# YyzHarry/imbalanced-regression

Measured on NVIDIA H100. Metric: images/sec, higher is better.
Workload: dtype bf16

## Files before the change

imbalanced-regression_b200/csrc/common.cuh:

```cuda
#pragma once
#include <cuda_runtime.h>
#include <cuda_bf16.h>
#include <stdint.h>
#include <stdio.h>
#include <stdlib.h>
#include <atomic>
#include <vector>
#include "../../include/dirb200.h"

namespace dirb200 {

void set_error(const char* fmt, ...);
extern std::atomic<int64_t> g_launches;

inline cudaStream_t as_stream(void* s) { return reinterpret_cast<cudaStream_t>(s); }

#define DIRB_CHECK_ARG(cond, ...)                \
  do {                                           \
    if (!(cond)) {                               \
      ::dirb200::set_error(__VA_ARGS__);         \
      return DIRB200_ERR_ARG;                    \
    }                                            \
  } while (0)

// ... 12 lines not shown
    DIRB_CUDA(cudaGetLastError());                \
  } while (0)

inline int num_sms() {
  static int n = 0;
  if (n == 0) {
    int dev = 0;
    if (cudaGetDevice(&dev) != cudaSuccess) return 132;
    if (cudaDeviceGetAttribute(&n, cudaDevAttrMultiProcessorCount, dev) != cudaSuccess || n <= 0) n = 132;
    if (const char* e = getenv("DIRB200_SMS")) {
      const int cap = atoi(e);
      if (cap > 0 && cap < n) n = cap;
    }
  }
  return n;
}

__device__ __forceinline__ float warp_sum(float v) {
#pragma unroll
  for (int o = 16; o > 0; o >>= 1) v += __shfl_xor_sync(0xffffffffu, v, o);
  return v;
}
__device__ __forceinline__ double warp_sum(double v) {
#pragma unroll
  for (int o = 16; o > 0; o >>= 1) v += __shfl_xor_sync(0xffffffffu, v, o);
  return v;
}

struct FastDiv {
  uint32_t mul, shr, d;
// ... 44 lines not shown
```

imbalanced-regression_b200/csrc/conv.cuh:

```cuda
#pragma once
#include "common.cuh"

namespace dirb200 {

struct ConvShape {
  int n, h, w, cin, cout, kh, kw, stride, pad, ho, wo;
};

struct StatLayout {
  int rows, n_tiles, bn, group;
};

int conv_fprop(const __nv_bfloat16* x, const __nv_bfloat16* w, __nv_bfloat16* y, const ConvShape& s, bool stem,
               cudaStream_t st, float* stat_partial = nullptr, StatLayout* layout = nullptr);
struct ConvEpilogue {
  const float* scale;
  const float* shift;
  const __nv_bfloat16* residual;
  bool relu;
};
int conv_fprop_affine(const __nv_bfloat16* x, const __nv_bfloat16* w, __nv_bfloat16* out, const ConvShape& s,
                      const ConvEpilogue& epi, cudaStream_t st);
struct DgradBnMoments {
  const __nv_bfloat16* y;
// ... 10 lines not shown
                        int* splits_out, cudaStream_t st);
int wgrad_reduce(const float* workspace, int splits, float* dw, const ConvShape& s, bool stem, bool accumulate,
                 cudaStream_t st);
int conv_wgrad(const __nv_bfloat16* x, const __nv_bfloat16* dy, float* dw, float* workspace, const ConvShape& s,
               bool stem, bool accumulate, cudaStream_t st);
struct WgradReduceDesc {
  const float* partial;
  size_t w_off;
  int splits, cout, cin, kh, kw, stem;
};
int wgrad_reduce_all(const WgradReduceDesc* descs_dev, int nlayers, float* grads, cudaStream_t st);
struct PrepDesc {
  size_t w_off;
  int cout, cin, kh, kw, stem;
  __nv_bfloat16 *wf, *wd;
  FastDiv fd_cin, fd_cout, fd_taps;
};
inline PrepDesc make_prep_desc(size_t w_off, int cout, int cin, int kh, int kw, int stem, __nv_bfloat16* wf,
                               __nv_bfloat16* wd) {
  PrepDesc d{w_off, cout, cin, kh, kw, stem, wf, wd, {}, {}, {}};
  d.fd_cin = make_fastdiv((uint32_t)cin);
  d.fd_cout = make_fastdiv((uint32_t)cout);
  d.fd_taps = make_fastdiv((uint32_t)(kh * kw));
  return d;
}
int conv_plan(const ConvShape& s, bool stem, int op, int* plan);
int prep_weights_all(const float* params, const PrepDesc* descs_dev, int nlayers, cudaStream_t st);
int prep_weights(const float* w, int cout, int cin, int kh, int kw, bool stem, __nv_bfloat16* wf, __nv_bfloat16* wd,
                 cudaStream_t st);
int input_to_s2d(const float* x, int n, int h, int w, __nv_bfloat16* out, cudaStream_t st);

}
```

imbalanced-regression_b200/csrc/conv_api.cu:

```cuda
#include "common.cuh"
#include "conv.cuh"

namespace dirb200 {

__global__ void prep_weights_kernel(const float* __restrict__ w, int cout, int cin, int kh, int kw,
                                    __nv_bfloat16* __restrict__ wf, __nv_bfloat16* __restrict__ wd) {
  const int64_t total = (int64_t)cout * cin * kh * kw;
  for (int64_t i = blockIdx.x * (int64_t)blockDim.x + threadIdx.x; i < total; i += (int64_t)gridDim.x * blockDim.x) {
    int c = (int)(i % cin);
    int64_t t = i / cin;
    int s = (int)(t % kw); t /= kw;
    int r = (int)(t % kh);
    int co = (int)(t / kh);
    const float v = w[(((int64_t)co * cin + c) * kh + r) * kw + s];
    const __nv_bfloat16 b = __float2bfloat16_rn(v);
    wf[i] = b;
    if (wd) wd[(((int64_t)c * kh + r) * kw + s) * cout + co] = b;
  }
}

__global__ void prep_stem_weights_kernel(const float* __restrict__ w, int cout, __nv_bfloat16* __restrict__ wf) {
  const int total = cout * 256;
  for (int i = blockIdx.x * blockDim.x + threadIdx.x; i < total; i += gridDim.x * blockDim.x) {
    const int co = i >> 8, k = i & 255;
    const int rp = k >> 6, sp = (k >> 4) & 3, ph = (k >> 3) & 1, pw = (k >> 2) & 1, c = k & 3;
    const int r = 2 * rp + ph - 1, s = 2 * sp + pw - 1;
    float v = 0.f;
    if (c < 3 && r >= 0 && s >= 0 && r < 7 && s < 7) v = w[((co * 3 + c) * 7 + r) * 7 + s];
    wf[i] = __float2bfloat16_rn(v);
  }
}

__global__ void input_to_s2d_kernel(const float* __restrict__ x, int n, int h, int w, __nv_bfloat16* __restrict__ out) {
  const int h2 = h / 2, w2 = w / 2;
  const int64_t total = (int64_t)n * h2 * w2;
  for (int64_t i = blockIdx.x * (int64_t)blockDim.x + threadIdx.x; i < total; i += (int64_t)gridDim.x * blockDim.x) {
    const int xw = (int)(i % w2);
    const int yh = (int)((i / w2) % h2);
    const int b = (int)(i / ((int64_t)w2 * h2));
    __align__(16) __nv_bfloat16 v[16];
#pragma unroll
    for (int ph = 0; ph < 2; ++ph)
#pragma unroll
      for (int pw = 0; pw < 2; ++pw) {
#pragma unroll
        for (int c = 0; c < 3; ++c)
          v[(ph * 2 + pw) * 4 + c] =
              __float2bfloat16_rn(x[(((int64_t)b * 3 + c) * h + (2 * yh + ph)) * w + (2 * xw + pw)]);
// ... 26 lines not shown
  const int total = 256 * cout;
  for (int i = blockIdx.x * blockDim.x + threadIdx.x; i < total; i += gridDim.x * blockDim.x) {
    const int co = i >> 8, k = i & 255;
    const int rp = k >> 6, sp_ = (k >> 4) & 3, ph = (k >> 3) & 1, pw = (k >> 2) & 1, c = k & 3;
    const int r = 2 * rp + ph - 1, s = 2 * sp_ + pw - 1;
    if (c >= 3 || r < 0 || s < 0) continue;
    float acc = 0.f;
    for (int sp = 0; sp < splits; ++sp) acc += partial[(int64_t)sp * total + i];
    float* o = dw + ((co * 3 + c) * 7 + r) * 7 + s;
    *o = accumulate ? *o + acc : acc;
  }
}

__global__ void __launch_bounds__(256)
wgrad_reduce_all_kernel(const WgradReduceDesc* __restrict__ descs, float* __restrict__ grads) {
  const WgradReduceDesc d = descs[blockIdx.y];
  float* dw = grads + d.w_off;
  if (d.stem) {
    const int total = 256 * d.cout;
    for (int i = blockIdx.x * blockDim.x + threadIdx.x; i < total; i += gridDim.x * blockDim.x) {
      const int co = i >> 8, k = i & 255;
      const int rp = k >> 6, sp_ = (k >> 4) & 3, ph = (k >> 3) & 1, pw = (k >> 2) & 1, c = k & 3;
      const int r = 2 * rp + ph - 1, s = 2 * sp_ + pw - 1;
      if (c >= 3 || r < 0 || s < 0) continue;
      float acc = 0.f;
      for (int sp = 0; sp < d.splits; ++sp) acc += d.partial[(int64_t)sp * total + i];
      dw[((co * 3 + c) * 7 + r) * 7 + s] += acc;
    }
    return;
  }
// ... 7 lines not shown
    for (; sp + 4 <= d.splits; sp += 4) {
      a0 += p[(int64_t)sp * total];
      a1 += p[(int64_t)(sp + 1) * total];
      a2 += p[(int64_t)(sp + 2) * total];
      a3 += p[(int64_t)(sp + 3) * total];
    }
    for (; sp < d.splits; ++sp) a0 += p[(int64_t)sp * total];
    const int64_t co = i / ktot, k = i - co * ktot;
    const int c = (int)(k % d.cin), t = (int)(k / d.cin);
    dw[(co * d.cin + c) * taps + t] += (a0 + a1) + (a2 + a3);
  }
}

int wgrad_reduce_all(const WgradReduceDesc* descs_dev, int nlayers, float* grads, cudaStream_t st) {
  if (nlayers <= 0) return DIRB200_OK;
  wgrad_reduce_all_kernel<<<dim3(2 * num_sms(), nlayers), 256, 0, st>>>(descs_dev, grads);
  DIRB_LAUNCHED();
  return DIRB200_OK;
}

__global__ void prep_weights_all_kernel(const float* __restrict__ params, const PrepDesc* __restrict__ descs) {
  const PrepDesc d = descs[blockIdx.y];
  const float* w = params + d.w_off;
  if (d.stem) {
    const int total = d.cout * 256;
    for (int i = blockIdx.x * blockDim.x + threadIdx.x; i < total; i += gridDim.x * blockDim.x) {
      const int co = i >> 8, k = i & 255;
      const int rp = k >> 6, sp = (k >> 4) & 3, ph = (k >> 3) & 1, pw = (k >> 2) & 1, c = k & 3;
      const int r = 2 * rp + ph - 1, s = 2 * sp + pw - 1;
      float v = 0.f;
      if (c < 3 && r >= 0 && s >= 0 && r < 7 && s < 7) v = w[((co * 3 + c) * 7 + r) * 7 + s];
      d.wf[i] = __float2bfloat16_rn(v);
    }
    return;
  }
  const uint32_t taps = (uint32_t)(d.kh * d.kw);
  const uint32_t total = (uint32_t)d.cout * (uint32_t)d.cin * taps;
  const uint32_t stride = gridDim.x * blockDim.x;
  for (uint32_t i = blockIdx.x * blockDim.x + threadIdx.x; i < total; i += stride) {
    uint32_t t, c, co, tap;
    d.fd_cin.divmod(i, t, c);
    d.fd_taps.divmod(t, co, tap);
    d.wf[i] = __float2bfloat16_rn(w[((size_t)co * d.cin + c) * taps + tap]);
  }
  if (!d.wd) return;
  for (uint32_t i = blockIdx.x * blockDim.x + threadIdx.x; i < total; i += stride) {
    uint32_t t, c, co, tap;
    d.fd_cout.divmod(i, t, co);
    d.fd_taps.divmod(t, c, tap);
    d.wd[i] = __float2bfloat16_rn(w[((size_t)co * d.cin + c) * taps + tap]);
  }
}

int prep_weights_all(const float* params, const PrepDesc* descs_dev, int nlayers, cudaStream_t st) {
  prep_weights_all_kernel<<<dim3(96, nlayers), 256, 0, st>>>(params, descs_dev);
  DIRB_LAUNCHED();
  return DIRB200_OK;
}

static inline int grid1d(int64_t n, int block = 256) {
  int64_t g = (n + block - 1) / block;
  const int64_t cap = 8 * (int64_t)num_sms();
  return (int)(g < 1 ? 1 : (g > cap ? cap : g));
}

int prep_weights(const float* w, int cout, int cin, int kh, int kw, bool stem, __nv_bfloat16* wf, __nv_bfloat16* wd,
                 cudaStream_t st) {
  if (stem) {
    prep_stem_weights_kernel<<<grid1d((int64_t)cout * 256), 256, 0, st>>>(w, cout, wf);
  } else {
    prep_weights_kernel<<<grid1d((int64_t)cout * cin * kh * kw), 256, 0, st>>>(w, cout, cin, kh, kw, wf, wd);
  }
  DIRB_LAUNCHED();
  return DIRB200_OK;
}

int input_to_s2d(const float* x, int n, int h, int w, __nv_bfloat16* out, cudaStream_t st) {
  input_to_s2d_kernel<<<grid1d((int64_t)n * (h / 2) * (w / 2)), 256, 0, st>>>(x, n, h, w, out);
  DIRB_LAUNCHED();
  return DIRB200_OK;
}

int wgrad_reduce(const float* workspace, int splits, float* dw, const ConvShape& s, bool stem, bool accumulate,
                 cudaStream_t st) {
  if (stem)
    wgrad_reduce_stem_kernel<<<grid1d(256 * (int64_t)s.cout), 256, 0, st>>>(workspace, splits, s.cout, accumulate, dw);
  else
  {
    const int64_t total = (int64_t)s.kh * s.kw * s.cin * s.cout;
    wgrad_reduce_kernel<<<(unsigned)((total + 255) / 256), 256, 0, st>>>(workspace, splits, s.cout, s.cin, s.kh, s.kw,
                                                                         accumulate, dw);
  }
  DIRB_LAUNCHED();
// ... 181 lines not shown
```

imbalanced-regression_b200/csrc/conv_igemm.cu:

```cuda
#include <stdlib.h>
#include "common.cuh"
#include "tc.cuh"
#include "conv.cuh"

namespace dirb200 {
using namespace tc;

constexpr int BM = 128;
constexpr int BK = 64;
constexpr int kProducerThreads = 128;
constexpr int kThreads = 384;
constexpr int kMaxTaps = 25;
constexpr int kMaxSmemBytes = 232448;

struct IgemmParams {
  const __nv_bfloat16* src;
  int n, hs, ws, cs;
  int hm, wm;
  int kh, kw, stride, pad;
  int transposed;
  int cls_on, cls_py, cls_px, full_h, full_w;
  int ntaps_c;
  int tap_list[kMaxTaps];
  long long tap_eoff[kMaxTaps];
// ... 133 lines not shown
    } else {
      split = 0;
      m_tile = t;
      n_tile = fixed_n;
      kb_begin = 0;
      nk = P.num_kblocks;
    }
  };

  if (threadIdx.x == 0) {
    for (int s = 0; s < C::kStages; ++s) {
      mbar_init(full_bar(s), ATMA ? 1 : kProducerThreads + 1);
      mbar_init(empty_bar(s), 8);
    }
    fence_barrier_init();
  }
  __syncthreads();

  if (warp < 4) {
    if constexpr (!ATMA) {
      const int j = lane & 7;
      const int q = lane >> 3;
      uint32_t rs = 0, rph = 0;
      for (int t = tile_first; t < tile_end; t += tile_step) {
        int split, m_tile, n_tile, kb_begin, nk;
        decode_tile(t, split, m_tile, n_tile, kb_begin, nk);
        const int n0 = n_tile * BN;
        long long off8[8];
        uint32_t mask8[8];
        int chunk_r = 0, chunk_s = 0, chunk_c0 = 0;
        bool chunk_ok = true;
        uint32_t tile_off = 0;
// ... 478 lines not shown
}

template <int BN, bool WGRAD, bool STEM, bool ATMA = false, bool AFFINE = false, bool BSTAT = false>
static int launch_igemm_impl(const CUtensorMap& tm, const CUtensorMap& tma, const IgemmParams& Qin, cudaStream_t st) {
  using C = Cfg<BN, !WGRAD>;
  const IgemmParams Q = finish_params(Qin);
  static bool configured = false;
  if (!configured) {
    DIRB_CUDA(cudaFuncSetAttribute(igemm_kernel<BN, WGRAD, STEM, ATMA, AFFINE, BSTAT>,
                                   cudaFuncAttributeMaxDynamicSharedMemorySize, C::kSmemBytes));
    configured = true;
  }
  int grid = Q.num_tiles < num_sms() ? Q.num_tiles : num_sms();
  if (!WGRAD && grid < Q.n_tiles) grid = Q.n_tiles;
  t_last_layout = StatLayout{grid, Q.n_tiles, BN, 1};
  igemm_kernel<BN, WGRAD, STEM, ATMA, AFFINE, BSTAT><<<grid, kThreads, C::kSmemBytes, st>>>(tm, tma, Q);
  DIRB_LAUNCHED();
  return DIRB200_OK;
}

template <int BN, bool WGRAD, bool STEM>
static int launch_igemm(const CUtensorMap& tm, const IgemmParams& P, int m_tiles, int splits, cudaStream_t st,
                        const CUtensorMap* tma = nullptr) {
  IgemmParams Q = P;
  Q.m_tiles = m_tiles;
  Q.num_tiles = m_tiles * P.n_tiles * splits;
  if constexpr (!STEM) {
    if (tma) {
      if constexpr (!WGRAD) {
        if (Q.epi_scale != nullptr) return launch_igemm_impl<BN, false, false, true, true>(tm, *tma, Q, st);
        if (Q.bst_y != nullptr) return launch_igemm_impl<BN, false, false, true, false, true>(tm, *tma, Q, st);
// ... 313 lines not shown
```

imbalanced-regression_b200/csrc/nn_kernels.cu:

```cuda
#include "common.cuh"
#include "conv.cuh"
#include "nn.cuh"

namespace dirb200 {

constexpr int kReduceCtasPerSm = 4;

struct V8 {
  float v[8];
};
__device__ __forceinline__ V8 load8(const __nv_bfloat16* p) {
  const uint4 u = *reinterpret_cast<const uint4*>(p);
  const __nv_bfloat162* h = reinterpret_cast<const __nv_bfloat162*>(&u);
  V8 r;
#pragma unroll
  for (int i = 0; i < 4; ++i) {
    const float2 f = __bfloat1622float2(h[i]);
    r.v[2 * i] = f.x;
    r.v[2 * i + 1] = f.y;
  }
  return r;
}
__device__ __forceinline__ void store8(__nv_bfloat16* p, const V8& a) {
  uint4 u;
// ... 122 lines not shown
  sh[1][threadIdx.y][threadIdx.x] = b0 + b1;
  __syncthreads();
  r0 = r1 = 0.0;
  if (threadIdx.y == 0)
    for (int w = 0; w < 32; ++w) {
      r0 += sh[0][w][threadIdx.x];
      r1 += sh[1][w][threadIdx.x];
    }
}

__global__ void bn_finalize_kernel(const float* __restrict__ partial, StatLayout L, int64_t rows, int c,
                                   const float* __restrict__ gamma, const float* __restrict__ beta, float eps,
                                   float momentum, float* __restrict__ running_mean, float* __restrict__ running_var,
                                   float* __restrict__ mean_out, float* __restrict__ invstd_out,
                                   float* __restrict__ scale, float* __restrict__ shift) {
  __shared__ double sh[2][32][32];
  const int i = blockIdx.x * 32 + threadIdx.x;
  double sx, sq;
  sum_layout2(partial, L, c, i, sh, sx, sq);
  if (threadIdx.y != 0 || i >= c) return;
  const double n = (double)rows;
  const double m = sx / n;
  double var = sq / n - m * m;
  if (var < 0.0) var = 0.0;
  const float invstd = (float)(1.0 / sqrt(var + (double)eps));
  mean_out[i] = (float)m;
  invstd_out[i] = invstd;
  const float sc = gamma[i] * invstd;
  scale[i] = sc;
  shift[i] = beta[i] - (float)m * sc;
// ... 23 lines not shown
  d.scale[i] = sc;
  d.shift[i] = params[d.beta_off + i] - running[d.rm_off + i] * sc;
}

__device__ __forceinline__ uint32_t f2_to_bf2(float a, float b) {
  __nv_bfloat162 h = __floats2bfloat162_rn(a, b);
  return *reinterpret_cast<uint32_t*>(&h);
}

template <bool HAS_RES, bool HAS_RESY, bool MASK>
__global__ void __launch_bounds__(256)
bn_apply_kernel(const __nv_bfloat16* __restrict__ y, const float* __restrict__ scale, const float* __restrict__ shift,
                const __nv_bfloat16* __restrict__ res, const __nv_bfloat16* __restrict__ res_y,
                const float* __restrict__ res_scale, const float* __restrict__ res_shift, int relu, int64_t rows,
                int c, __nv_bfloat16* __restrict__ out, uint8_t* __restrict__ mask_out) {
  constexpr int R = (HAS_RES || HAS_RESY) ? 2 : 4;
  const int cgroups = c / 8;
  const int cg = threadIdx.x % cgroups, lane = threadIdx.x / cgroups, lanes = blockDim.x / cgroups;
  const V8 sc = loadf8(scale + cg * 8), sh = loadf8(shift + cg * 8);
  V8 rs{}, rh{};
  if (HAS_RESY) {
    rs = loadf8(res_scale + cg * 8);
    rh = loadf8(res_shift + cg * 8);
  }
  const int64_t stride = (int64_t)gridDim.x * lanes;
  for (int64_t r0 = blockIdx.x * (int64_t)lanes + lane; r0 < rows; r0 += R * stride) {
    int64_t offs[R], rr[R];
    bool live[R];
    uint4 Y[R], RV[R];
#pragma unroll
// ... 80 lines not shown
    hw.divmod(static_cast<uint32_t>(r), n, rem);
    w.divmod(rem, yy, xx);
    r2 = (static_cast<int64_t>(n) * h2 + (yy >> 1)) * w2 + (xx >> 1);
    return ((yy | xx) & 1u) == 0u;
  }
};

template <int MODE, int G2M, bool HAS_Y2, bool WRITE_DZ, bool HAS_G3 = false>
__global__ void __launch_bounds__(256, 3)
bn_bwd_reduce_kernel(const __nv_bfloat16* __restrict__ g1, const __nv_bfloat16* __restrict__ g2, CompactG2 cg2,
                     const __nv_bfloat16* __restrict__ g3, const __nv_bfloat16* __restrict__ y,
                     const __nv_bfloat16* __restrict__ y2,
                     const float* __restrict__ scale, const float* __restrict__ shift,
                     const uint8_t* __restrict__ mask, int64_t rows, int c, float* __restrict__ partial,
                     __nv_bfloat16* __restrict__ dz_out) {
  constexpr bool HAS_G2 = G2M != G2_NONE;
  const int cgroups = c / 8;
  const int cg = threadIdx.x % cgroups, lane = threadIdx.x / cgroups, lanes = blockDim.x / cgroups;
  constexpr int K = HAS_Y2 ? 3 : 2;
  float acc[K][8] = {};
  MaskSrc<MODE> ms;
  ms.init(scale, shift, mask, cgroups, cg);
  const int64_t stride = (int64_t)gridDim.x * lanes;
  for (int64_t r0 = blockIdx.x * (int64_t)lanes + lane; r0 < rows; r0 += 2 * stride) {
    const int64_t r1 = r0 + stride;
    const bool two = r1 < rows;
    const int64_t o0 = r0 * c + cg * 8, o1 = (two ? r1 : r0) * c + cg * 8;
    uint4 G[2], Y[2], G2[2], Y2[2], G3[2];
    uint32_t M[2];
    G[0] = *reinterpret_cast<const uint4*>(g1 + o0);
// ... 67 lines not shown
                                                    const float* __restrict__ gamma, float* __restrict__ grad_gamma,
                                                    float* __restrict__ grad_beta, float* __restrict__ coef) {
  const double n = (double)rows, is = (double)invstd[i], ga = (double)gamma[i], mu = (double)mean[i];
  const double dg = is * (s1 - mu * db);
  coef[i] = (float)(ga * is);
  coef[c + i] = (float)(-ga * is * is * dg / n);
  coef[2 * c + i] = (float)(ga * is * (mu * is * dg / n - db / n));
  grad_gamma[i] += (float)dg;
  grad_beta[i] += (float)db;
}

__global__ void bn_bwd_coeffs_kernel(const float* __restrict__ partial, int nblocks, int K, int gslot, int64_t rows,
                                     int c, const float* __restrict__ mean, const float* __restrict__ invstd,
                                     const float* __restrict__ gamma, float* __restrict__ grad_gamma,
                                     float* __restrict__ grad_beta, float* __restrict__ coef ) {
  __shared__ double sh[32][32];
  const int i = blockIdx.x * 32 + threadIdx.x;
  double db, s1;
  sum_partials2(partial, nblocks, K, 0, gslot, c, i, sh, db, s1);
  if (threadIdx.y != 0 || i >= c) return;
  bn_bwd_coeffs_write(db, s1, i, rows, c, mean, invstd, gamma, grad_gamma, grad_beta, coef);
}

__global__ void bn_bwd_coeffs_layout_kernel(const float* __restrict__ partial, StatLayout L, int64_t rows, int c,
                                            const float* __restrict__ mean, const float* __restrict__ invstd,
                                            const float* __restrict__ gamma, float* __restrict__ grad_gamma,
                                            float* __restrict__ grad_beta, float* __restrict__ coef) {
  __shared__ double sh[2][32][32];
  const int i = blockIdx.x * 32 + threadIdx.x;
  double db, s1;
  sum_layout2(partial, L, c, i, sh, db, s1);
  if (threadIdx.y != 0 || i >= c) return;
  bn_bwd_coeffs_write(db, s1, i, rows, c, mean, invstd, gamma, grad_gamma, grad_beta, coef);
}

template <int MODE, int G2M, bool HAS_Y2, bool WRITE_DZ>
__global__ void __launch_bounds__(256, 2)
bn_bwd_apply_kernel(const __nv_bfloat16* __restrict__ g1, const __nv_bfloat16* __restrict__ g2, CompactG2 cg2,
                    const __nv_bfloat16* __restrict__ y, const float* __restrict__ coef,
                    const __nv_bfloat16* __restrict__ y2, const float* __restrict__ coef2,
                    const float* __restrict__ scale, const float* __restrict__ shift,
                    const uint8_t* __restrict__ mask, int64_t rows, int c, __nv_bfloat16* __restrict__ dy,
                    __nv_bfloat16* __restrict__ dy2, __nv_bfloat16* __restrict__ dz_out) {
  constexpr bool HAS_G2 = G2M != G2_NONE;
  constexpr int R = (HAS_G2 || HAS_Y2) ? 2 : 4;
  const int cgroups = c / 8;
  const int cg = threadIdx.x % cgroups, lane = threadIdx.x / cgroups, lanes = blockDim.x / cgroups;
  const V8 A = loadf8(coef + cg * 8), B = loadf8(coef + c + cg * 8), C = loadf8(coef + 2 * c + cg * 8);
  V8 A2{}, B2{}, C2{};
  if (HAS_Y2) {
    A2 = loadf8(coef2 + cg * 8);
    B2 = loadf8(coef2 + c + cg * 8);
    C2 = loadf8(coef2 + 2 * c + cg * 8);
  }
  MaskSrc<MODE> ms;
  ms.init(scale, shift, mask, cgroups, cg);
  const int64_t stride = (int64_t)gridDim.x * lanes;
  for (int64_t r0 = blockIdx.x * (int64_t)lanes + lane; r0 < rows; r0 += R * stride) {
// ... 83 lines not shown
    }
    V8 o;
    __align__(8) uint8_t ib[8];
#pragma unroll
    for (int j = 0; j < 8; ++j) { o.v[j] = best[j]; ib[j] = (uint8_t)bi[j]; }
    const int64_t off = (((int64_t)b * ho + yo) * wo + xo) * c + g * 8;
    store8(out + off, o);
    *reinterpret_cast<uint2*>(idx + off) = *reinterpret_cast<uint2*>(ib);
  }
}

__global__ void __launch_bounds__(256)
bn_relu_maxpool_fwd_kernel(const __nv_bfloat16* __restrict__ y, const float* __restrict__ scale,
                           const float* __restrict__ shift, int n, int h, int w, int c,
                           __nv_bfloat16* __restrict__ out, uint8_t* __restrict__ idx) {
  const int ho = (h + 2 - 3) / 2 + 1, wo = (w + 2 - 3) / 2 + 1, cg = c / 8;
  const int hb = (ho + 1) / 2, wb = (wo + 1) / 2;
  const int64_t total = (int64_t)n * hb * wb * cg;
  for (int64_t i = blockIdx.x * (int64_t)blockDim.x + threadIdx.x; i < total; i += (int64_t)gridDim.x * blockDim.x) {
    const int g = (int)(i % cg);
    int64_t t = i / cg;
    const int xb = (int)(t % wb); t /= wb;
    const int yb = (int)(t % hb);
    const int b = (int)(t / hb);
    const V8 sc = loadf8(scale + g * 8), sh = loadf8(shift + g * 8);
    uint32_t best[4][8];
#pragma unroll
    for (int k = 0; k < 4; ++k)
#pragma unroll
      for (int j = 0; j < 8; ++j) best[k][j] = 0u;
// ... 50 lines not shown
        uint32_t ow[4], iw[2] = {0u, 0u};
#pragma unroll
        for (int p = 0; p < 4; ++p) ow[p] = (bk[2 * p] >> 4) | ((bk[2 * p + 1] >> 4) << 16);
#pragma unroll
        for (int j = 0; j < 8; ++j) iw[j >> 2] |= (15u - (bk[j] & 15u)) << (8 * (j & 3));
        const int64_t off = (((int64_t)b * ho + yo) * wo + xo) * c + g * 8;
        *reinterpret_cast<uint4*>(out + off) = make_uint4(ow[0], ow[1], ow[2], ow[3]);
        *reinterpret_cast<uint2*>(idx + off) = make_uint2(iw[0], iw[1]);
      }
  }
}

__global__ void __launch_bounds__(256)
maxpool_bwd_kernel(const __nv_bfloat16* __restrict__ g1, const __nv_bfloat16* __restrict__ g2,
                   const uint8_t* __restrict__ idx, int n, int h, int w, int c, __nv_bfloat16* __restrict__ dx) {
  const int ho = (h + 2 - 3) / 2 + 1, wo = (w + 2 - 3) / 2 + 1, cg = c / 8;
  const int hb = h / 2, wb = w / 2;
  const int64_t total = (int64_t)n * hb * wb * cg;
  for (int64_t i = blockIdx.x * (int64_t)blockDim.x + threadIdx.x; i < total; i += (int64_t)gridDim.x * blockDim.x) {
    const int g = (int)(i % cg);
    int64_t t = i / cg;
    const int xb = (int)(t % wb); t /= wb;
    const int ya = (int)(t % hb);
    const int b = (int)(t / hb);
    uint4 gv[4], g2v[4];
    uint2 iv[4];
    bool ok[4];
#pragma unroll
    for (int k = 0; k < 4; ++k) {
      const int yo = ya + (k >> 1), xo = xb + (k & 1);
// ... 29 lines not shown
            if (ib[2 * j] == pos) acc[py * 2 + px].v[2 * j] += f.x;
            if (ib[2 * j + 1] == pos) acc[py * 2 + px].v[2 * j + 1] += f.y;
          }
        }
      }
    }
#pragma unroll
    for (int py = 0; py < 2; ++py)
#pragma unroll
      for (int px = 0; px < 2; ++px)
        store8(dx + ((((int64_t)b * h + 2 * ya + py) * w + 2 * xb + px) * c + g * 8), acc[py * 2 + px]);
  }
}

__global__ void avgpool_fwd_kernel(const __nv_bfloat16* __restrict__ x, int n, int hw, int c, float* __restrict__ enc) {
  const int cg = c / 8;
  const int64_t total = (int64_t)n * cg;
  for (int64_t i = blockIdx.x * (int64_t)blockDim.x + threadIdx.x; i < total; i += (int64_t)gridDim.x * blockDim.x) {
    const int g = (int)(i % cg);
    const int b = (int)(i / cg);
    float acc[8] = {};
    for (int p = 0; p < hw; ++p) {
      const V8 v = load8(x + ((int64_t)b * hw + p) * c + g * 8);
#pragma unroll
      for (int j = 0; j < 8; ++j) acc[j] += v.v[j];
    }
    const float inv = 1.f / (float)hw;
#pragma unroll
    for (int j = 0; j < 8; ++j) enc[(int64_t)b * c + g * 8 + j] = acc[j] * inv;
  }
}

__global__ void avgpool_bwd_kernel(const float* __restrict__ genc, int n, int hw, int c, __nv_bfloat16* __restrict__ dx) {
  const int cg = c / 8;
  const int64_t total = (int64_t)n * hw * cg;
  const float inv = 1.f / (float)hw;
  for (int64_t i = blockIdx.x * (int64_t)blockDim.x + threadIdx.x; i < total; i += (int64_t)gridDim.x * blockDim.x) {
    const int g = (int)(i % cg);
    const int b = (int)(i / ((int64_t)cg * hw));
    V8 o = loadf8(genc + (int64_t)b * c + g * 8);
#pragma unroll
    for (int j = 0; j < 8; ++j) o.v[j] *= inv;
    store8(dx + i * 8, o);
  }
}

__global__ void __launch_bounds__(256) linear1_fwd_kernel(const float* __restrict__ x, const float* __restrict__ w,
                                                          const float* __restrict__ bias, int d,
// ... 319 lines not shown
  DIRB_CHECK_ARG(rows > 0, "bn_stats: rows must be positive");
  const int cgroups = c / 8;
  const int lanes = 256 / cgroups;
  *nblocks = reduce_grid(rows, lanes);
  bn_stats_kernel<<<*nblocks, 256, 256 * 16 * sizeof(float), st>>>(y, rows, c, partial);
  DIRB_LAUNCHED();
  return DIRB200_OK;
}

int bn_finalize(const float* partial, const StatLayout& layout, int64_t rows, int c, const float* gamma,
                const float* beta, float eps, float momentum, float* running_mean, float* running_var, float* mean,
                float* invstd, float* scale, float* shift, cudaStream_t st) {
  DIRB_CHECK_ARG(layout.rows > 0 && layout.n_tiles > 0 && layout.bn > 0 && layout.group > 0 &&
                     layout.n_tiles * layout.bn >= c,
                 "bn_finalize: bad statistics layout");
  bn_finalize_kernel<<<(c + 31) / 32, dim3(32, 32), 0, st>>>(partial, layout, rows, c, gamma, beta, eps, momentum,
                                                             running_mean, running_var, mean, invstd, scale, shift);
  DIRB_LAUNCHED();
  return DIRB200_OK;
}

int bn_eval_coeffs(int c, const float* gamma, const float* beta, float eps, const float* running_mean,
                   const float* running_var, float* scale, float* shift, cudaStream_t st) {
  bn_eval_coeffs_kernel<<<(c + 127) / 128, 128, 0, st>>>(c, gamma, beta, eps, running_mean, running_var, scale, shift);
  DIRB_LAUNCHED();
  return DIRB200_OK;
}

int bn_eval_coeffs_all(const BnEvalDesc* descs_dev, int nlayers, int max_c, const float* params, const float* running,
                       float eps, cudaStream_t st) {
  bn_eval_coeffs_all_kernel<<<dim3((max_c + 255) / 256, nlayers), 256, 0, st>>>(descs_dev, params, running, eps);
  DIRB_LAUNCHED();
// ... 1 lines not shown
}

int bn_apply(const __nv_bfloat16* y, const float* scale, const float* shift, const __nv_bfloat16* res,
             const __nv_bfloat16* res_y, const float* res_scale, const float* res_shift, bool relu, int64_t rows, int c,
             __nv_bfloat16* out, uint8_t* mask_out, cudaStream_t st) {
  DIRB_CHECK_ARG(bn_channels_ok(c), "bn_apply: unsupported channel count %d (8, 16, 32, ..., 2048)", c);
  DIRB_CHECK_ARG(rows > 0, "bn_apply: rows must be positive");
  const int cgroups = c / 8;
  DIRB_CHECK_ARG(!(res && res_y), "bn_apply: one shortcut operand (identity or the downsample branch's raw output)");
  DIRB_CHECK_ARG(!mask_out || relu, "bn_apply: the ReLU mask needs relu");
  const int want = stream_grid(rows, 256 / cgroups);
#define DIRB_BNA(RES, RESY, MASK)                                                                                 \
  do {                                                                                                            \
    static const int occ = resident_ctas(bn_apply_kernel<RES, RESY, MASK>, 0);                                    \
    const int grid = want < occ * num_sms() ? want : occ * num_sms();                                             \
    bn_apply_kernel<RES, RESY, MASK><<<grid, 256, 0, st>>>(y, scale, shift, res, res_y, res_scale, res_shift,     \
                                                           relu ? 1 : 0, rows, c, out, mask_out);                 \
  } while (0)
  if (res && mask_out) DIRB_BNA(true, false, true);
  else if (res) DIRB_BNA(true, false, false);
  else if (res_y && mask_out) DIRB_BNA(false, true, true);
  else if (res_y) DIRB_BNA(false, true, false);
  else if (mask_out) DIRB_BNA(false, false, true);
  else DIRB_BNA(false, false, false);
#undef DIRB_BNA
  DIRB_LAUNCHED();
  return DIRB200_OK;
}

static CompactG2 make_compact(int g2_h, int g2_w) {
  CompactG2 cg{};
  if (g2_h > 0 && g2_w > 0) {
// ... 12 lines not shown
  DIRB_CHECK_ARG(!g3 || (g2 && dz_out), "bn_bwd_reduce: a third gradient is added in the two-gradient identity forms only");
  DIRB_CHECK_ARG(bn_channels_ok(c), "bn_bwd_reduce: unsupported channel count %d (8, 16, 32, ..., 2048)", c);
  DIRB_CHECK_ARG(rows > 0, "bn_bwd_reduce: rows must be positive");
  DIRB_CHECK_ARG(compact_ok(g2_h, g2_w, rows) && (g2_h == 0 || (g2 && mask && !y2)),
                 "bn_bwd_reduce: bad compact second gradient");
  const int cgroups = c / 8;
  DIRB_CHECK_ARG(mask || (!g2 && !y2 && (scale != nullptr) == (shift != nullptr)),
                 "bn_bwd_reduce: the mask-from-y and the no-ReLU forms take one gradient, one BN");
  DIRB_CHECK_ARG(!dz_out || (mask && !y2), "bn_bwd_reduce: dz is stored for identity blocks only");
  const int lanes = 256 / cgroups;
  const size_t smem = 256 * (y2 ? 24 : 16) * sizeof(float);
#define DIRB_RED3(MODE, G2, Y2, DZ, G3)                                                                             \
  do {                                                                                                              \
    static const int occ = resident_ctas(bn_bwd_reduce_kernel<MODE, G2, Y2, DZ, G3>, 256 * 24 * sizeof(float));     \
    *nblocks = reduce_grid(rows, lanes, occ);                                                                       \
    bn_bwd_reduce_kernel<MODE, G2, Y2, DZ, G3><<<*nblocks, 256, smem, st>>>(g1, g2, cg2, g3, y, y2, scale, shift, mask, \
                                                                            rows, c, partial, dz_out);              \
  } while (0)
#define DIRB_RED(MODE, G2, Y2, DZ) DIRB_RED3(MODE, G2, Y2, DZ, false)
  if (g3 && g2_h) DIRB_RED3(MASK_BITS, G2_COMPACT, false, true, true);
  else if (g3) DIRB_RED3(MASK_BITS, G2_DENSE, false, true, true);
  else if (!mask && !scale) DIRB_RED(MASK_NONE, G2_NONE, false, false);
  else if (!mask) DIRB_RED(MASK_FROM_Y, G2_NONE, false, false);
  else if (g2_h && dz_out) DIRB_RED(MASK_BITS, G2_COMPACT, false, true);
  else if (g2_h) DIRB_RED(MASK_BITS, G2_COMPACT, false, false);
  else if (g2 && y2) DIRB_RED(MASK_BITS, G2_DENSE, true, false);
  else if (g2 && dz_out) DIRB_RED(MASK_BITS, G2_DENSE, false, true);
  else if (g2) DIRB_RED(MASK_BITS, G2_DENSE, false, false);
  else if (y2) DIRB_RED(MASK_BITS, G2_NONE, true, false);
  else if (dz_out) DIRB_RED(MASK_BITS, G2_NONE, false, true);
  else DIRB_RED(MASK_BITS, G2_NONE, false, false);
#undef DIRB_RED
#undef DIRB_RED3
  DIRB_LAUNCHED();
  return DIRB200_OK;
}

int bn_bwd_coeffs(const float* partial, int nblocks, int k, int gslot, int64_t rows, int c, const float* mean,
                  const float* invstd, const float* gamma, float* grad_gamma, float* grad_beta, float* coef,
                  cudaStream_t st) {
  bn_bwd_coeffs_kernel<<<(c + 31) / 32, dim3(32, 32), 0, st>>>(partial, nblocks, k, gslot, rows, c, mean, invstd, gamma,
                                                      grad_gamma, grad_beta, coef);
  DIRB_LAUNCHED();
  return DIRB200_OK;
}

int bn_bwd_coeffs_layout(const float* partial, const StatLayout& layout, int64_t rows, int c, const float* mean,
                         const float* invstd, const float* gamma, float* grad_gamma, float* grad_beta, float* coef,
                         cudaStream_t st) {
  DIRB_CHECK_ARG(layout.rows > 0 && layout.n_tiles > 0 && layout.bn > 0 && layout.group > 0 &&
                     layout.n_tiles * layout.bn >= c,
                 "bn_bwd_coeffs_layout: bad partial layout");
  bn_bwd_coeffs_layout_kernel<<<(c + 31) / 32, dim3(32, 32), 0, st>>>(partial, layout, rows, c, mean, invstd, gamma,
                                                                      grad_gamma, grad_beta, coef);
  DIRB_LAUNCHED();
  return DIRB200_OK;
}

int bn_bwd_apply(const __nv_bfloat16* g1, const __nv_bfloat16* g2, const __nv_bfloat16* y, const float* coef,
                 const __nv_bfloat16* y2, const float* coef2, const float* scale, const float* shift,
                 const uint8_t* mask, int64_t rows, int c, __nv_bfloat16* dy, __nv_bfloat16* dy2,
                 __nv_bfloat16* dz_out, cudaStream_t st, int g2_h, int g2_w) {
  const CompactG2 cg2 = make_compact(g2_h, g2_w);
  DIRB_CHECK_ARG(bn_channels_ok(c), "bn_bwd_apply: unsupported channel count %d (8, 16, 32, ..., 2048)", c);
  DIRB_CHECK_ARG(rows > 0, "bn_bwd_apply: rows must be positive");
  DIRB_CHECK_ARG(compact_ok(g2_h, g2_w, rows) && (g2_h == 0 || (g2 && mask && !y2 && dz_out)),
                 "bn_bwd_apply: bad compact second gradient");
  const int cgroups = c / 8;
  DIRB_CHECK_ARG(mask || (!g2 && !y2 && !dz_out && (scale != nullptr) == (shift != nullptr)),
                 "bn_bwd_apply: the mask-from-y and the dz-input forms take one gradient, one BN");
  DIRB_CHECK_ARG(!(y2 && dz_out), "bn_bwd_apply: a block has either a downsample branch or an identity path");
  const int want = stream_grid(rows, 256 / cgroups);
#define DIRB_APP(MODE, G2, Y2, DZ)                                                                                     \
  do {                                                                                                                 \
    static const int occ = resident_ctas(bn_bwd_apply_kernel<MODE, G2, Y2, DZ>, 0);                                    \
    const int grid = want < occ * num_sms() ? want : occ * num_sms();                                                  \
    bn_bwd_apply_kernel<MODE, G2, Y2, DZ><<<grid, 256, 0, st>>>(g1, g2, cg2, y, coef, y2, coef2, scale, shift, mask, rows, \
                                                               c, dy, dy2, dz_out);                                    \
  } while (0)
  if (!mask && !scale) DIRB_APP(MASK_NONE, G2_NONE, false, false);
  else if (!mask) DIRB_APP(MASK_FROM_Y, G2_NONE, false, false);
  else if (g2_h) DIRB_APP(MASK_BITS, G2_COMPACT, false, true);
  else if (g2 && y2) DIRB_APP(MASK_BITS, G2_DENSE, true, false);
  else if (g2 && dz_out) DIRB_APP(MASK_BITS, G2_DENSE, false, true);
  else if (g2) DIRB_APP(MASK_BITS, G2_DENSE, false, false);
  else if (y2) DIRB_APP(MASK_BITS, G2_NONE, true, false);
  else if (dz_out) DIRB_APP(MASK_BITS, G2_NONE, false, true);
  else DIRB_APP(MASK_BITS, G2_NONE, false, false);
#undef DIRB_APP
  DIRB_LAUNCHED();
  return DIRB200_OK;
}

int maxpool_fwd(const __nv_bfloat16* x, int n, int h, int w, int c, __nv_bfloat16* out, uint8_t* idx, cudaStream_t st) {
  const int ho = (h - 1) / 2 + 1, wo = (w - 1) / 2 + 1;
  maxpool_fwd_kernel<<<grid1d((int64_t)n * ho * wo * c / 8), 256, 0, st>>>(x, n, h, w, c, out, idx);
  DIRB_LAUNCHED();
  return DIRB200_OK;
}

int bn_relu_maxpool_fwd(const __nv_bfloat16* y, const float* scale, const float* shift, int n, int h, int w, int c,
                        __nv_bfloat16* out, uint8_t* idx, cudaStream_t st) {
  const int ho = (h - 1) / 2 + 1, wo = (w - 1) / 2 + 1;
  bn_relu_maxpool_fwd_kernel<<<grid1d((int64_t)n * ((ho + 1) / 2) * ((wo + 1) / 2) * c / 8), 256, 0, st>>>(y, scale, shift, n, h, w, c,
                                                                                                out, idx);
  DIRB_LAUNCHED();
  return DIRB200_OK;
}

int maxpool_bwd(const __nv_bfloat16* g1, const __nv_bfloat16* g2, const uint8_t* idx, int n, int h, int w, int c,
                __nv_bfloat16* dx, cudaStream_t st) {
  DIRB_CHECK_ARG(h % 2 == 0 && w % 2 == 0, "maxpool_bwd: H and W must be even");
  maxpool_bwd_kernel<<<grid1d((int64_t)n * (h / 2) * (w / 2) * c / 8), 256, 0, st>>>(g1, g2, idx, n, h, w, c, dx);
  DIRB_LAUNCHED();
  return DIRB200_OK;
}

int avgpool_fwd(const __nv_bfloat16* x, int n, int hw, int c, float* enc, cudaStream_t st) {
  avgpool_fwd_kernel<<<grid1d((int64_t)n * c / 8, 128), 128, 0, st>>>(x, n, hw, c, enc);
  DIRB_LAUNCHED();
  return DIRB200_OK;
}

int avgpool_bwd(const float* genc, int n, int hw, int c, __nv_bfloat16* dx, cudaStream_t st) {
  avgpool_bwd_kernel<<<grid1d((int64_t)n * hw * c / 8), 256, 0, st>>>(genc, n, hw, c, dx);
  DIRB_LAUNCHED();
  return DIRB200_OK;
}

}

using namespace dirb200;

extern "C" {

size_t dirb200_bn_workspace_bytes(int c) { return sizeof(float) * static_cast<size_t>(bn_partial_floats(c)); }

int dirb200_bn_train_fwd(const void* y, int64_t rows, int c, const float* gamma, const float* beta, float eps,
                         float momentum, float* running_mean, float* running_var, int relu, void* out, float* save_mean,
                         float* save_invstd, float* scale_shift, void* workspace, void* stream) {
// ... 353 lines not shown
```

Measured before the change: 7682.

## Enable programmatic dependent launch across kernels and tile-transpose dgrad weight prep

Launches most conv, BN, pooling and weight-prep kernels with programmatic stream serialization and puts griddepcontrol.wait at the start of each kernel. The next kernel's launch and prologue (barrier init, tensormap prefetch) can then overlap the tail of the previous one. Separately, it replaces the strided divmod gather for dgrad weights with a 32x32 shared-memory tile transpose so both reads and writes are coalesced. It also adds tensormap prefetch in the igemm kernel. Because no kernel issues an explicit trigger, the overlap is limited to launch latency, and any kernel missing the wait could race.

```diff
diff --git a/imbalanced-regression_b200/csrc/common.cuh b/imbalanced-regression_b200/csrc/common.cuh
--- a/imbalanced-regression_b200/csrc/common.cuh
+++ b/imbalanced-regression_b200/csrc/common.cuh
@@ -5,6 +5,7 @@
 #include <stdio.h>
 #include <stdlib.h>
 #include <atomic>
+#include <utility>
 #include <vector>
 #include "../../include/dirb200.h"
 
@@ -50,6 +51,24 @@
     }
   }
   return n;
+}
+
+__device__ __forceinline__ void pdl_wait() { asm volatile("griddepcontrol.wait;" ::: "memory"); }
+
+template <typename... KArgs, typename... Args>
+inline cudaError_t launch_pdl(void (*kernel)(KArgs...), dim3 grid, dim3 block, size_t smem, cudaStream_t st,
+                              Args&&... args) {
+  cudaLaunchAttribute attr[1];
+  attr[0].id = cudaLaunchAttributeProgrammaticStreamSerialization;
+  attr[0].val.programmaticStreamSerializationAllowed = 1;
+  cudaLaunchConfig_t cfg{};
+  cfg.gridDim = grid;
+  cfg.blockDim = block;
+  cfg.dynamicSmemBytes = smem;
+  cfg.stream = st;
+  cfg.attrs = attr;
+  cfg.numAttrs = 1;
+  return cudaLaunchKernelEx(&cfg, kernel, std::forward<Args>(args)...);
 }
 
 __device__ __forceinline__ float warp_sum(float v) {
diff --git a/imbalanced-regression_b200/csrc/conv.cuh b/imbalanced-regression_b200/csrc/conv.cuh
--- a/imbalanced-regression_b200/csrc/conv.cuh
+++ b/imbalanced-regression_b200/csrc/conv.cuh
@@ -48,13 +48,12 @@
   size_t w_off;
   int cout, cin, kh, kw, stem;
   __nv_bfloat16 *wf, *wd;
-  FastDiv fd_cin, fd_cout, fd_taps;
+  FastDiv fd_cin, fd_taps;
 };
 inline PrepDesc make_prep_desc(size_t w_off, int cout, int cin, int kh, int kw, int stem, __nv_bfloat16* wf,
                                __nv_bfloat16* wd) {
-  PrepDesc d{w_off, cout, cin, kh, kw, stem, wf, wd, {}, {}, {}};
+  PrepDesc d{w_off, cout, cin, kh, kw, stem, wf, wd, {}, {}};
   d.fd_cin = make_fastdiv((uint32_t)cin);
-  d.fd_cout = make_fastdiv((uint32_t)cout);
   d.fd_taps = make_fastdiv((uint32_t)(kh * kw));
   return d;
 }
diff --git a/imbalanced-regression_b200/csrc/conv_api.cu b/imbalanced-regression_b200/csrc/conv_api.cu
--- a/imbalanced-regression_b200/csrc/conv_api.cu
+++ b/imbalanced-regression_b200/csrc/conv_api.cu
@@ -32,6 +32,7 @@
 }
 
 __global__ void input_to_s2d_kernel(const float* __restrict__ x, int n, int h, int w, __nv_bfloat16* __restrict__ out) {
+  pdl_wait();
   const int h2 = h / 2, w2 = w / 2;
   const int64_t total = (int64_t)n * h2 * w2;
   for (int64_t i = blockIdx.x * (int64_t)blockDim.x + threadIdx.x; i < total; i += (int64_t)gridDim.x * blockDim.x) {
@@ -88,6 +89,7 @@
 
 __global__ void __launch_bounds__(256)
 wgrad_reduce_all_kernel(const WgradReduceDesc* __restrict__ descs, float* __restrict__ grads) {
+  pdl_wait();
   const WgradReduceDesc d = descs[blockIdx.y];
   float* dw = grads + d.w_off;
   if (d.stem) {
@@ -125,12 +127,13 @@
 
 int wgrad_reduce_all(const WgradReduceDesc* descs_dev, int nlayers, float* grads, cudaStream_t st) {
   if (nlayers <= 0) return DIRB200_OK;
-  wgrad_reduce_all_kernel<<<dim3(2 * num_sms(), nlayers), 256, 0, st>>>(descs_dev, grads);
+  DIRB_CUDA(launch_pdl(wgrad_reduce_all_kernel, dim3(2 * num_sms(), nlayers), dim3(256), 0, st, descs_dev, grads));
   DIRB_LAUNCHED();
   return DIRB200_OK;
 }
 
 __global__ void prep_weights_all_kernel(const float* __restrict__ params, const PrepDesc* __restrict__ descs) {
+  pdl_wait();
   const PrepDesc d = descs[blockIdx.y];
   const float* w = params + d.w_off;
   if (d.stem) {
@@ -155,16 +158,29 @@
     d.wf[i] = __float2bfloat16_rn(w[((size_t)co * d.cin + c) * taps + tap]);
   }
   if (!d.wd) return;
-  for (uint32_t i = blockIdx.x * blockDim.x + threadIdx.x; i < total; i += stride) {
-    uint32_t t, c, co, tap;
-    d.fd_cout.divmod(i, t, co);
-    d.fd_taps.divmod(t, c, tap);
-    d.wd[i] = __float2bfloat16_rn(w[((size_t)co * d.cin + c) * taps + tap]);
+  __shared__ float tile[32][33];
+  const int ktot = d.cin * (int)taps;
+  const int tiles_k = (ktot + 31) / 32, tiles = ((d.cout + 31) / 32) * tiles_k;
+  const int tx = threadIdx.x & 31, ty = threadIdx.x >> 5;
+  for (int t = blockIdx.x; t < tiles; t += gridDim.x) {
+    const int co0 = (t / tiles_k) * 32, k0 = (t % tiles_k) * 32;
+#pragma unroll
+    for (int j = 0; j < 32; j += 8) {
+      const int co = co0 + ty + j, k = k0 + tx;
+      if (co < d.cout && k < ktot) tile[ty + j][tx] = w[(size_t)co * ktot + k];
+    }
+    __syncthreads();
+#pragma unroll
+    for (int j = 0; j < 32; j += 8) {
+      const int k = k0 + ty + j, co = co0 + tx;
+      if (co < d.cout && k < ktot) d.wd[(size_t)k * d.cout + co] = __float2bfloat16_rn(tile[tx][ty + j]);
+    }
+    __syncthreads();
   }
 }
 
 int prep_weights_all(const float* params, const PrepDesc* descs_dev, int nlayers, cudaStream_t st) {
-  prep_weights_all_kernel<<<dim3(96, nlayers), 256, 0, st>>>(params, descs_dev);
+  DIRB_CUDA(launch_pdl(prep_weights_all_kernel, dim3(96, nlayers), dim3(256), 0, st, params, descs_dev));
   DIRB_LAUNCHED();
   return DIRB200_OK;
 }
@@ -187,7 +203,8 @@
 }
 
 int input_to_s2d(const float* x, int n, int h, int w, __nv_bfloat16* out, cudaStream_t st) {
-  input_to_s2d_kernel<<<grid1d((int64_t)n * (h / 2) * (w / 2)), 256, 0, st>>>(x, n, h, w, out);
+  DIRB_CUDA(launch_pdl(input_to_s2d_kernel, dim3(grid1d((int64_t)n * (h / 2) * (w / 2))), dim3(256), 0, st, x, n, h, w,
+                       out));
   DIRB_LAUNCHED();
   return DIRB200_OK;
 }
diff --git a/imbalanced-regression_b200/csrc/conv_igemm.cu b/imbalanced-regression_b200/csrc/conv_igemm.cu
--- a/imbalanced-regression_b200/csrc/conv_igemm.cu
+++ b/imbalanced-regression_b200/csrc/conv_igemm.cu
@@ -171,8 +171,11 @@
       mbar_init(empty_bar(s), 8);
     }
     fence_barrier_init();
+    asm volatile("prefetch.tensormap [%0];" ::"l"(&tmap_b) : "memory");
+    if constexpr (ATMA) asm volatile("prefetch.tensormap [%0];" ::"l"(&tmap_a) : "memory");
   }
   __syncthreads();
+  pdl_wait();
 
   if (warp < 4) {
     if constexpr (!ATMA) {
@@ -681,7 +684,8 @@
   int grid = Q.num_tiles < num_sms() ? Q.num_tiles : num_sms();
   if (!WGRAD && grid < Q.n_tiles) grid = Q.n_tiles;
   t_last_layout = StatLayout{grid, Q.n_tiles, BN, 1};
-  igemm_kernel<BN, WGRAD, STEM, ATMA, AFFINE, BSTAT><<<grid, kThreads, C::kSmemBytes, st>>>(tm, tma, Q);
+  DIRB_CUDA(launch_pdl(igemm_kernel<BN, WGRAD, STEM, ATMA, AFFINE, BSTAT>, dim3(grid), dim3(kThreads), C::kSmemBytes, st,
+                       tm, tma, Q));
   DIRB_LAUNCHED();
   return DIRB200_OK;
 }
diff --git a/imbalanced-regression_b200/csrc/nn_kernels.cu b/imbalanced-regression_b200/csrc/nn_kernels.cu
--- a/imbalanced-regression_b200/csrc/nn_kernels.cu
+++ b/imbalanced-regression_b200/csrc/nn_kernels.cu
@@ -160,6 +160,7 @@
                                    float momentum, float* __restrict__ running_mean, float* __restrict__ running_var,
                                    float* __restrict__ mean_out, float* __restrict__ invstd_out,
                                    float* __restrict__ scale, float* __restrict__ shift) {
+  pdl_wait();
   __shared__ double sh[2][32][32];
   const int i = blockIdx.x * 32 + threadIdx.x;
   double sx, sq;
@@ -213,6 +214,7 @@
                 const __nv_bfloat16* __restrict__ res, const __nv_bfloat16* __restrict__ res_y,
                 const float* __restrict__ res_scale, const float* __restrict__ res_shift, int relu, int64_t rows,
                 int c, __nv_bfloat16* __restrict__ out, uint8_t* __restrict__ mask_out) {
+  pdl_wait();
   constexpr int R = (HAS_RES || HAS_RESY) ? 2 : 4;
   const int cgroups = c / 8;
   const int cg = threadIdx.x % cgroups, lane = threadIdx.x / cgroups, lanes = blockDim.x / cgroups;
@@ -323,6 +325,7 @@
                      const float* __restrict__ scale, const float* __restrict__ shift,
                      const uint8_t* __restrict__ mask, int64_t rows, int c, float* __restrict__ partial,
                      __nv_bfloat16* __restrict__ dz_out) {
+  pdl_wait();
   constexpr bool HAS_G2 = G2M != G2_NONE;
   const int cgroups = c / 8;
   const int cg = threadIdx.x % cgroups, lane = threadIdx.x / cgroups, lanes = blockDim.x / cgroups;
@@ -420,6 +423,7 @@
                                      int c, const float* __restrict__ mean, const float* __restrict__ invstd,
                                      const float* __restrict__ gamma, float* __restrict__ grad_gamma,
                                      float* __restrict__ grad_beta, float* __restrict__ coef ) {
+  pdl_wait();
   __shared__ double sh[32][32];
   const int i = blockIdx.x * 32 + threadIdx.x;
   double db, s1;
@@ -432,6 +436,7 @@
                                             const float* __restrict__ mean, const float* __restrict__ invstd,
                                             const float* __restrict__ gamma, float* __restrict__ grad_gamma,
                                             float* __restrict__ grad_beta, float* __restrict__ coef) {
+  pdl_wait();
   __shared__ double sh[2][32][32];
   const int i = blockIdx.x * 32 + threadIdx.x;
   double db, s1;
@@ -448,6 +453,7 @@
                     const float* __restrict__ scale, const float* __restrict__ shift,
                     const uint8_t* __restrict__ mask, int64_t rows, int c, __nv_bfloat16* __restrict__ dy,
                     __nv_bfloat16* __restrict__ dy2, __nv_bfloat16* __restrict__ dz_out) {
+  pdl_wait();
   constexpr bool HAS_G2 = G2M != G2_NONE;
   constexpr int R = (HAS_G2 || HAS_Y2) ? 2 : 4;
   const int cgroups = c / 8;
@@ -561,6 +567,7 @@
 bn_relu_maxpool_fwd_kernel(const __nv_bfloat16* __restrict__ y, const float* __restrict__ scale,
                            const float* __restrict__ shift, int n, int h, int w, int c,
                            __nv_bfloat16* __restrict__ out, uint8_t* __restrict__ idx) {
+  pdl_wait();
   const int ho = (h + 2 - 3) / 2 + 1, wo = (w + 2 - 3) / 2 + 1, cg = c / 8;
   const int hb = (ho + 1) / 2, wb = (wo + 1) / 2;
   const int64_t total = (int64_t)n * hb * wb * cg;
@@ -641,6 +648,7 @@
 __global__ void __launch_bounds__(256)
 maxpool_bwd_kernel(const __nv_bfloat16* __restrict__ g1, const __nv_bfloat16* __restrict__ g2,
                    const uint8_t* __restrict__ idx, int n, int h, int w, int c, __nv_bfloat16* __restrict__ dx) {
+  pdl_wait();
   const int ho = (h + 2 - 3) / 2 + 1, wo = (w + 2 - 3) / 2 + 1, cg = c / 8;
   const int hb = h / 2, wb = w / 2;
   const int64_t total = (int64_t)n * hb * wb * cg;
@@ -700,6 +708,7 @@
 }
 
 __global__ void avgpool_fwd_kernel(const __nv_bfloat16* __restrict__ x, int n, int hw, int c, float* __restrict__ enc) {
+  pdl_wait();
   const int cg = c / 8;
   const int64_t total = (int64_t)n * cg;
   for (int64_t i = blockIdx.x * (int64_t)blockDim.x + threadIdx.x; i < total; i += (int64_t)gridDim.x * blockDim.x) {
@@ -718,6 +727,7 @@
 }
 
 __global__ void avgpool_bwd_kernel(const float* __restrict__ genc, int n, int hw, int c, __nv_bfloat16* __restrict__ dx) {
+  pdl_wait();
   const int cg = c / 8;
   const int64_t total = (int64_t)n * hw * cg;
   const float inv = 1.f / (float)hw;
@@ -1067,8 +1077,8 @@
   DIRB_CHECK_ARG(layout.rows > 0 && layout.n_tiles > 0 && layout.bn > 0 && layout.group > 0 &&
                      layout.n_tiles * layout.bn >= c,
                  "bn_finalize: bad statistics layout");
-  bn_finalize_kernel<<<(c + 31) / 32, dim3(32, 32), 0, st>>>(partial, layout, rows, c, gamma, beta, eps, momentum,
-                                                             running_mean, running_var, mean, invstd, scale, shift);
+  DIRB_CUDA(launch_pdl(bn_finalize_kernel, dim3((c + 31) / 32), dim3(32, 32), 0, st, partial, layout, rows, c, gamma, beta,
+                       eps, momentum, running_mean, running_var, mean, invstd, scale, shift));
   DIRB_LAUNCHED();
   return DIRB200_OK;
 }
@@ -1100,8 +1110,8 @@
   do {                                                                                                            \
     static const int occ = resident_ctas(bn_apply_kernel<RES, RESY, MASK>, 0);                                    \
     const int grid = want < occ * num_sms() ? want : occ * num_sms();                                             \
-    bn_apply_kernel<RES, RESY, MASK><<<grid, 256, 0, st>>>(y, scale, shift, res, res_y, res_scale, res_shift,     \
-                                                           relu ? 1 : 0, rows, c, out, mask_out);                 \
+    DIRB_CUDA(launch_pdl(bn_apply_kernel<RES, RESY, MASK>, dim3(grid), dim3(256), 0, st, y, scale, shift, res, res_y, \
+                         res_scale, res_shift, relu ? 1 : 0, rows, c, out, mask_out));                            \
   } while (0)
   if (res && mask_out) DIRB_BNA(true, false, true);
   else if (res) DIRB_BNA(true, false, false);
@@ -1144,8 +1154,8 @@
   do {                                                                                                              \
     static const int occ = resident_ctas(bn_bwd_reduce_kernel<MODE, G2, Y2, DZ, G3>, 256 * 24 * sizeof(float));     \
     *nblocks = reduce_grid(rows, lanes, occ);                                                                       \
-    bn_bwd_reduce_kernel<MODE, G2, Y2, DZ, G3><<<*nblocks, 256, smem, st>>>(g1, g2, cg2, g3, y, y2, scale, shift, mask, \
-                                                                            rows, c, partial, dz_out);              \
+    DIRB_CUDA(launch_pdl(bn_bwd_reduce_kernel<MODE, G2, Y2, DZ, G3>, dim3(*nblocks), dim3(256), smem, st, g1, g2, cg2, \
+                         g3, y, y2, scale, shift, mask, rows, c, partial, dz_out));                                 \
   } while (0)
 #define DIRB_RED(MODE, G2, Y2, DZ) DIRB_RED3(MODE, G2, Y2, DZ, false)
   if (g3 && g2_h) DIRB_RED3(MASK_BITS, G2_COMPACT, false, true, true);
@@ -1169,8 +1179,8 @@
 int bn_bwd_coeffs(const float* partial, int nblocks, int k, int gslot, int64_t rows, int c, const float* mean,
                   const float* invstd, const float* gamma, float* grad_gamma, float* grad_beta, float* coef,
                   cudaStream_t st) {
-  bn_bwd_coeffs_kernel<<<(c + 31) / 32, dim3(32, 32), 0, st>>>(partial, nblocks, k, gslot, rows, c, mean, invstd, gamma,
-                                                      grad_gamma, grad_beta, coef);
+  DIRB_CUDA(launch_pdl(bn_bwd_coeffs_kernel, dim3((c + 31) / 32), dim3(32, 32), 0, st, partial, nblocks, k, gslot, rows, c,
+                       mean, invstd, gamma, grad_gamma, grad_beta, coef));
   DIRB_LAUNCHED();
   return DIRB200_OK;
 }
@@ -1181,8 +1191,8 @@
   DIRB_CHECK_ARG(layout.rows > 0 && layout.n_tiles > 0 && layout.bn > 0 && layout.group > 0 &&
                      layout.n_tiles * layout.bn >= c,
                  "bn_bwd_coeffs_layout: bad partial layout");
-  bn_bwd_coeffs_layout_kernel<<<(c + 31) / 32, dim3(32, 32), 0, st>>>(partial, layout, rows, c, mean, invstd, gamma,
-                                                                      grad_gamma, grad_beta, coef);
+  DIRB_CUDA(launch_pdl(bn_bwd_coeffs_layout_kernel, dim3((c + 31) / 32), dim3(32, 32), 0, st, partial, layout, rows, c,
+                       mean, invstd, gamma, grad_gamma, grad_beta, coef));
   DIRB_LAUNCHED();
   return DIRB200_OK;
 }
@@ -1205,8 +1215,8 @@
   do {                                                                                                                 \
     static const int occ = resident_ctas(bn_bwd_apply_kernel<MODE, G2, Y2, DZ>, 0);                                    \
     const int grid = want < occ * num_sms() ? want : occ * num_sms();                                                  \
-    bn_bwd_apply_kernel<MODE, G2, Y2, DZ><<<grid, 256, 0, st>>>(g1, g2, cg2, y, coef, y2, coef2, scale, shift, mask, rows, \
-                                                               c, dy, dy2, dz_out);                                    \
+    DIRB_CUDA(launch_pdl(bn_bwd_apply_kernel<MODE, G2, Y2, DZ>, dim3(grid), dim3(256), 0, st, g1, g2, cg2, y, coef, y2, \
+                         coef2, scale, shift, mask, rows, c, dy, dy2, dz_out));                                        \
   } while (0)
   if (!mask && !scale) DIRB_APP(MASK_NONE, G2_NONE, false, false);
   else if (!mask) DIRB_APP(MASK_FROM_Y, G2_NONE, false, false);
@@ -1232,8 +1242,8 @@
 int bn_relu_maxpool_fwd(const __nv_bfloat16* y, const float* scale, const float* shift, int n, int h, int w, int c,
                         __nv_bfloat16* out, uint8_t* idx, cudaStream_t st) {
   const int ho = (h - 1) / 2 + 1, wo = (w - 1) / 2 + 1;
-  bn_relu_maxpool_fwd_kernel<<<grid1d((int64_t)n * ((ho + 1) / 2) * ((wo + 1) / 2) * c / 8), 256, 0, st>>>(y, scale, shift, n, h, w, c,
-                                                                                                out, idx);
+  const int grid = grid1d((int64_t)n * ((ho + 1) / 2) * ((wo + 1) / 2) * c / 8);
+  DIRB_CUDA(launch_pdl(bn_relu_maxpool_fwd_kernel, dim3(grid), dim3(256), 0, st, y, scale, shift, n, h, w, c, out, idx));
   DIRB_LAUNCHED();
   return DIRB200_OK;
 }
@@ -1241,19 +1251,20 @@
 int maxpool_bwd(const __nv_bfloat16* g1, const __nv_bfloat16* g2, const uint8_t* idx, int n, int h, int w, int c,
                 __nv_bfloat16* dx, cudaStream_t st) {
   DIRB_CHECK_ARG(h % 2 == 0 && w % 2 == 0, "maxpool_bwd: H and W must be even");
-  maxpool_bwd_kernel<<<grid1d((int64_t)n * (h / 2) * (w / 2) * c / 8), 256, 0, st>>>(g1, g2, idx, n, h, w, c, dx);
+  const int grid = grid1d((int64_t)n * (h / 2) * (w / 2) * c / 8);
+  DIRB_CUDA(launch_pdl(maxpool_bwd_kernel, dim3(grid), dim3(256), 0, st, g1, g2, idx, n, h, w, c, dx));
   DIRB_LAUNCHED();
   return DIRB200_OK;
 }
 
 int avgpool_fwd(const __nv_bfloat16* x, int n, int hw, int c, float* enc, cudaStream_t st) {
-  avgpool_fwd_kernel<<<grid1d((int64_t)n * c / 8, 128), 128, 0, st>>>(x, n, hw, c, enc);
+  DIRB_CUDA(launch_pdl(avgpool_fwd_kernel, dim3(grid1d((int64_t)n * c / 8, 128)), dim3(128), 0, st, x, n, hw, c, enc));
   DIRB_LAUNCHED();
   return DIRB200_OK;
 }
 
 int avgpool_bwd(const float* genc, int n, int hw, int c, __nv_bfloat16* dx, cudaStream_t st) {
-  avgpool_bwd_kernel<<<grid1d((int64_t)n * hw * c / 8), 256, 0, st>>>(genc, n, hw, c, dx);
+  DIRB_CUDA(launch_pdl(avgpool_bwd_kernel, dim3(grid1d((int64_t)n * hw * c / 8)), dim3(256), 0, st, genc, n, hw, c, dx));
   DIRB_LAUNCHED();
   return DIRB200_OK;
 }
```

Result: no change. 7731, median of 6 (+0.6%).
